# MisterVVP/poor-man-s-cache

Hardware: AMD Instinct MI355X
Metric: device-resident value compress+decompress GiB/s at 1/2/4/8 MI355X (higher is better)
Workload: dtype u8; 1 GPU; 10000000 x 1024 B values per GPU (JSON-slice), batched gzip level-9 compress + decompress, device-resident; outputs not checked in this run (--full checks every member); partition=MurmurHash3_x64_128('key'+i)[0] % 128 % n_gpus (NUM_SHARDS=128), parallelism=shard-partitioned x1, no collective

## Files before the change

poor-man-s-cache_amd/csrc/pmc_capi.hip:

```cpp
#include <hip/hip_runtime.h>

#include <vector>

#include <algorithm>
#include <atomic>
#include <cstdlib>
#include <cstdio>
#include <cstring>
#include <chrono>
#include <condition_variable>
#include <functional>
#include <mutex>
#include <string>
#include <thread>

#include <unistd.h>

#include "../../include/pmc_codec.h"
#include "pmc_device.hpp"
#include "pmc_kernels.hpp"

#define PMC_API extern "C" __attribute__((visibility("default")))

namespace pmc {
// ... 794 lines not shown
        e.cap_len = R.maxlen;
        e.wave_bytes = deflate_lv_emit_wave_bytes(R.maxlen);
        const uint64_t ew = std::max<uint64_t>(4, std::min<uint64_t>(
            {(uint64_t)(R.nv + 3) / 4 * 4, (uint64_t)ctx->cus * 4, std::max<uint64_t>(4, (8ull << 30) / e.wave_bytes / 4 * 4)}));
        r = ctx->lvemit.ensure(ew * e.wave_bytes);
        if (r) return r;
        e.scratch = (uint8_t *)ctx->lvemit.p;
        klaunch(ctx, PMC_K_DEFLATE_LARGE_EMIT, st, [&] {
            hipLaunchKernelGGL(deflate_lv_emit_kernel, dim3((unsigned)(ew / 4)), dim3(256), deflate_lv_emit_lds(4), st, e,
                               L);
        });
        hipError_t err = hipGetLastError();
        if (err != hipSuccess) {
            set_err(fast ? "fast large-value kernels" : "large-value kernels", err);
            return PMC_E_NO_DEVICE;
        }
        v0 = R.v1;
    }
    return PMC_OK;
}

static uint64_t split_chunk_budget() {
    static const uint64_t budget = (getenv("PMC_SPLIT_CHUNK_MB") ? (uint64_t)atoll(getenv("PMC_SPLIT_CHUNK_MB"))
                                                                 : 98304ull) << 20;
    return budget;
}

static int run_split_pass(pmc_ctx *ctx, DeflateArgs &a, const SplitPass &ps, uint32_t dD, hipStream_t st) {
    const uint64_t n = a.n, pcap = ps.pcap;
    const bool fastp = ps.fastp, dictp = ps.dictp;
    static const bool no_order = getenv("PMC_TREES_ORDER") && !atoi(getenv("PMC_TREES_ORDER"));
    const size_t tl_small = (size_t)(kTreesCap + 1) * 64 * 4, tl_1k = (size_t)(kTreesCap1K + 1) * 64 * 4;
    const size_t tl_big = (size_t)(kLCodes + 1) * 64 * 4;
    const uint32_t fcap = dictp ? 0u : front_cap_class(pcap);
    const uint64_t dcap = std::min<uint64_t>(((uint64_t)dD + ps.hi + 63) & ~(uint64_t)63, kDictSpan);
    const uint64_t fwb = dictp   ? deflate_front_fast_wave_bytes(dcap)
                         : fastp ? deflate_front_fast_wave_bytes(fcap ? fcap : pcap)
                                 : deflate_front_wave_bytes(fcap ? fcap : pcap);
    const uint64_t bwb = deflate_back_wave_bytes(pcap);
    a.dict = dictp ? (const uint8_t *)ctx->dict.p : nullptr;
    a.dict_len = dictp ? dD : 0u;
    a.front_cap = dictp ? (uint32_t)dcap : 0u;
    a.mtime = dictp ? ctx->dict_id : 0u;
    a.xfl = fastp ? 4u : 2u;
    const DeflateKernel fk = front_kernel(dictp, fastp, fcap);
    const Launch Lf = plan_lds(ctx, (const void *)fk, fwb, n, 0);
    const Launch Lb = plan_lds(ctx, (const void *)deflate_back_kernel, bwb, n, kBackTabBytes);
    const uint64_t chunk = split_chunk_of(n, split_chunk_budget(), pcap);
    const SplitLayout SL(pcap, chunk);
    uint8_t *p = (uint8_t *)ctx->split.p;
    a.cT = (uint32_t *)(p + SL.cT);
    a.cN = (uint32_t *)(p + SL.cN);
    a.cP = (uint32_t *)(p + SL.cP);
    a.cG = (uint32_t *)(p + SL.cG);
    a.cH = (uint16_t *)(p + SL.cH);
    a.cL = p + SL.cL;
    a.cB = (uint32_t *)(p + SL.cB);
    a.cC = (uint32_t *)(p + SL.cC);
    a.cD = (uint32_t *)(p + SL.cD);
    a.cZ = (uint32_t *)(p + SL.cZ);
    uint32_t *ord = (uint32_t *)(p + SL.ord), *obins = (uint32_t *)(p + SL.obins);
    a.cQ = (uint32_t *)(p + SL.cQ);
    a.min_len = ps.lo;
    a.lds_max_len = ps.hi;
    a.cap_len = pcap;
    a.front_batch = pcap <= 512 ? 4u : pcap <= 2048 ? 2u : 1u;
    for (uint64_t first = 0; first < n; first += chunk) {
        a.first = first;
        a.count = std::min<uint64_t>(chunk, n - first);
        const unsigned tb = (unsigned)((a.count + 63) / 64);
        a.wave_bytes = fwb;
        if (hipMemsetAsync(a.cQ, 0, 8, st) != hipSuccess) return PMC_E_NO_DEVICE;
        klaunch(ctx, PMC_K_DEFLATE_FRONT, st, [&] {
            const dim3 fg((unsigned)std::min<uint64_t>(Lf.blocks, (a.count + Lf.wpb - 1) / Lf.wpb));
            hipLaunchKernelGGL(fk, fg, dim3(64 * Lf.wpb), Lf.lds, st, a);
        });
        if (hipMemsetAsync(a.cD + a.count, 0, 4, st) != hipSuccess) return PMC_E_NO_DEVICE;
        a.cO = nullptr;
        if (!no_order && a.count >= 4096) {
            if (hipMemsetAsync(obins, 0, kOrderBins * 4, st) != hipSuccess) return PMC_E_NO_DEVICE;
            const unsigned ob = (unsigned)std::min<uint64_t>((a.count + 1023) / 1024, (uint64_t)ctx->cus * 4);
            klaunch(ctx, PMC_K_ORDER, st, [&] {
                hipLaunchKernelGGL(order_hist_kernel, dim3(ob), dim3(256), 0, st, (const uint32_t *)a.cZ, a.count, obins);
                hipLaunchKernelGGL(order_scan_kernel, dim3(1), dim3(1024), 0, st, obins);
                hipLaunchKernelGGL(order_scatter_kernel, dim3(ob), dim3(256), 0, st, (const uint32_t *)a.cZ, a.count,
                                   obins, ord);
            });
            a.cO = ord;
        }
        klaunch(ctx, PMC_K_DEFLATE_TREES, st, [&] {
            if (pcap <= 1024) hipLaunchKernelGGL(deflate_trees_kernel<kTreesCap1K>, dim3(tb), dim3(64), tl_1k, st, a);
            else hipLaunchKernelGGL(deflate_trees_kernel<kTreesCap>, dim3(tb), dim3(64), tl_small, st, a);
            hipLaunchKernelGGL(deflate_trees_kernel<kLCodes>, dim3(std::min<unsigned>(tb, 2u * (unsigned)ctx->cus)),
                               dim3(64), tl_big, st, a);
        });
        a.wave_bytes = bwb;
        a.back_nostage = pcap <= kNostageMaxLen ? 1u : 0u;
        if (a.back_nostage) klaunch(ctx, PMC_K_DEFLATE_BACK, st, [&] {
            const unsigned cb = (unsigned)std::min<uint64_t>((a.count + 511) / 512, (uint64_t)ctx->cus * 4);
            hipLaunchKernelGGL(crc32_batch_kernel, dim3(cb), dim3(512), 0, st, (const uint8_t *)a.src,
                               (const uint64_t *)(a.src_off + a.first), (const uint32_t *)(a.src_len + a.first),
                               a.count, a.cC);
        });
        klaunch(ctx, PMC_K_DEFLATE_BACK, st, [&] {
            hipLaunchKernelGGL(deflate_back_kernel,
                               dim3((unsigned)std::min<uint64_t>(Lb.blocks, (a.count + Lb.wpb - 1) / Lb.wpb)),
                               dim3(64 * Lb.wpb), Lb.lds, st, a);
// ... 1294 lines not shown
```

poor-man-s-cache_amd/csrc/pmc_deflate_split.hip:

```cpp
#include <hip/hip_runtime.h>

#include "pmc_device.hpp"
#include "pmc_kernels.hpp"

namespace pmc {


template <uint32_t CAPC>
__global__ void __launch_bounds__(256, 7) deflate_front_kernel(DeflateArgs a) {
    extern __shared__ __attribute__((aligned(16))) uint8_t lds[];
    const int wpb = blockDim.x / 64, wib = threadIdx.x / 64, l = lane_id();
    const uint64_t lcap = CAPC ? (uint64_t)CAPC : a.cap_len;
    uint8_t *base = lds + (uint64_t)wib * (CAPC ? front_layout(lcap).total : a.wave_bytes);
    const SmallLayout L = small_layout(lcap);
    const FrontLayout F = front_layout(lcap);
    SmallWave w;
    small_wave_init(w, base, L, a, nullptr);
    w.S = to_lds<uint16_t>(base + F.S);
    w.R = to_lds<uint16_t>(base + F.R);
    w.CN = to_lds<uint8_t>(base + F.cn);
    w.HC = to_lds<uint64_t>(base + F.hc);
    w.EV = to_lds<uint32_t>(base + F.ev);
    w.cnp = F.pkb;
    w.s12 = front_s12(lcap) ? 1u : 0u;
    w.lfreq = to_lds<uint32_t>(base + F.freq);
    w.dfreq = w.lfreq + 288;
    w.blfreq = w.dfreq + 32;
    const uint32_t kBatch = a.front_batch;
    uint32_t nx = l == 0 ? atomicAdd(a.cQ, kBatch) : 0u;
    for (;;) {
        const uint64_t g = readlane(nx, 0);
        if (g >= a.count) break;
        nx = l == 0 ? atomicAdd(a.cQ, kBatch) : 0u;
        const uint64_t vl = g + (uint64_t)l;
        const bool in = (uint32_t)l < kBatch && vl < a.count;
        const uint32_t myl = in ? a.src_len[a.first + vl] : 0u;
        const uint64_t myo = in ? a.src_off[a.first + vl] : 0u;
        uint64_t todo = ballot(myl != 0 && myl > a.min_len && myl <= a.lds_max_len);
        while (todo) {
            const int jj = __builtin_ctzll(todo);
            todo &= todo - 1;
            const uint64_t v = g + (uint64_t)jj, gv = a.first + v;
            const uint32_t len = readlane(myl, jj);
            w.tok = (PMC_GLB uint32_t *)(a.cT + v * a.cap_len);
#ifdef PMC_FAULT_LANE_ORDER
            w.fault_rev = (uint32_t)(gv & 1);
#endif
            const uint8_t *vsrc = a.src + readlane64(myo, jj);
            const uint32_t ntok = w.run_front(vsrc, len);
            if (ntok == kNtokRetry) {
                if (l == 0) {
                    a.cN[v] = kNtokRetry;
                    a.cZ[v] = 0;
                    atomicAdd(a.guard, 1u);
                }
                continue;
            }
            uint32_t nz = 0;
            for (int s = l; s < kLCodes + kDCodes; s += 64) {
                const uint32_t f = s < kLCodes ? w.lfreq[s] : w.dfreq[s - kLCodes];
                a.cH[v * kSplitRows + s] = (uint16_t)f;
                nz += (uint32_t)__builtin_popcountll(ballot(s < kLCodes && f != 0));
            }
            if (l == 0) {
                a.cN[v] = ntok < kSymsPerBlock ? ntok : kNtokMultiBlock;
                a.cZ[v] = nz;
            }
        }
    }
    small_wave_stamps_out(w, a);
}
template __global__ void deflate_front_kernel<0>(DeflateArgs);
template __global__ void deflate_front_kernel<1024>(DeflateArgs);
template __global__ void deflate_front_kernel<4096>(DeflateArgs);

template <int CAP>
struct LaneTrees {
    PMC_LDS uint32_t *hp;
    RegU16<kMaxBits + 1> blc;
    RegU16<kBLCodes> blf;
    const uint16_t *hist;
    uint8_t *lens;
    uint32_t *mg;
    bool deferred = false;

    __device__ uint32_t H(uint32_t i) const { return hp[i * 64]; }
    __device__ void setH(uint32_t i, uint32_t v) { hp[i * 64] = v; }

    __device__ void down(uint32_t k, uint32_t n) {
        const uint32_t v = H(k), kv = v >> 10;
        uint32_t j = k << 1;
        while (j <= n) {
            uint32_t x = H(j);
            if (j < n) {
                const uint32_t y = H(j + 1);
                if ((y >> 10) <= (x >> 10)) {
                    j++;
                    x = y;
                }
            }
            if (kv <= (x >> 10)) break;
            setH(k, x);
            k = j;
            j <<= 1;
        }
        setH(k, v);
    }

    __device__ static uint32_t xbits(int kind, uint32_t x) {
        return kind == 0 ? (x >= kLiterals + 1 ? len_extra_cf(x - (kLiterals + 1)) : 0u)
               : kind == 1 ? dist_extra_cf(x)
                           : (x == 16 ? 2u : x == 17 ? 3u : x == 18 ? 7u : 0u);
    }
    __device__ static uint32_t static_len(int kind, uint32_t x) {
        return kind == 1 ? 5u : x < 144 ? 8u : x < 256 ? 9u : x < 280 ? 7u : 8u;
    }
    template <class Freq>
    __device__ int build(Freq freq, int elems, uint32_t row0, int kind, int max_length, uint32_t &opt, uint32_t &stat,
                         PMC_GLB const uint16_t *grow = nullptr) {
        int heap_len = 0, max_code = -1;
        if (grow) {
            typedef uint32_t v4u __attribute__((ext_vector_type(4)));
            PMC_GLB const v4u *g4 = (PMC_GLB const v4u *)grow;
            const int nb = (elems + 31) / 32;
            v4u cur[4], nxt[4];
#pragma unroll
            for (int i = 0; i < 4; i++) cur[i] = i * 8 < elems ? g4[i] : v4u{0, 0, 0, 0};
            for (int b = 0; b < nb; b++) {
#pragma unroll
                for (int i = 0; i < 4; i++) {
                    const int q = (b + 1) * 4 + i;
                    nxt[i] = b + 1 < nb && q * 8 < elems ? g4[q] : v4u{0, 0, 0, 0};
                }
#pragma unroll
                for (int i = 0; i < 4; i++) {
#pragma unroll
                    for (int h = 0; h < 8; h++) {
                        const int nn = b * 32 + i * 8 + h;
                        const uint32_t f = nn < elems ? (cur[i][h >> 1] >> (16 * (h & 1))) & 0xffffu : 0u;
                        if (f) {
                            if (heap_len == CAP) {
                                deferred = true;
                                return -1;
                            }
                            setH(++heap_len, f << 15 | (uint32_t)nn);
                            max_code = nn;
                        }
                    }
                }
#pragma unroll
                for (int i = 0; i < 4; i++) cur[i] = nxt[i];
            }
        }
        for (int n0 = 0; !grow && n0 < elems; n0 += 8) {
            uint32_t f8[8];
#pragma unroll
            for (int k = 0; k < 8; k++) f8[k] = n0 + k < elems ? freq(n0 + k) : 0u;
#pragma unroll
            for (int k = 0; k < 8; k++) {
                if (f8[k]) {
                    if (heap_len == CAP) {
                        deferred = true;
                        return -1;
                    }
                    setH(++heap_len, f8[k] << 15 | (uint32_t)(n0 + k));
                    max_code = n0 + k;
                }
            }
        }
        while (heap_len < 2) {
            const int node = max_code < 2 ? ++max_code : 0;
            setH(++heap_len, 1u << 15 | (uint32_t)node);
            opt--;
            if (kind != 2) stat -= static_len(kind, (uint32_t)node);
        }
        for (int n = heap_len / 2; n >= 1; n--) down((uint32_t)n, (uint32_t)heap_len);
        uint32_t node = (uint32_t)elems, nm = 0;
        do {
            const uint32_t n = H(1);
            setH(1, H((uint32_t)heap_len));
            heap_len--;
            down(1, (uint32_t)heap_len);
            const uint32_t m = H(1);
            mg[(2 * nm) * 64] = n;
            mg[(2 * nm + 1) * 64] = m;
            nm++;
            const uint32_t kn = n >> 10, km = m >> 10, dn = kn & 31, dm = km & 31;
            const uint32_t d = (dn >= dm ? dn : dm) + 1;
            setH(1, ((((kn >> 5) + (km >> 5)) << 5) | d) << 10 | node);
            node++;
            down(1, (uint32_t)heap_len);
        } while (heap_len >= 2);
        const uint32_t K = nm;
        uint32_t overflow = 0;
        blc.zero();
        setH(K, 0);
        constexpr int kB = 8;
        uint32_t cur[2 * kB], nxt[2 * kB], nx2[2 * kB];
        auto fetch = [&](int hi, uint32_t *d) {
#pragma unroll
            for (int t = 0; t < kB; t++) {
                const int j = hi - 1 - t;
                d[2 * t] = j >= 0 ? mg[(2 * j + 1) * 64] : 0u;
                d[2 * t + 1] = j >= 0 ? mg[(2 * j) * 64] : 0u;
            }
        };
        fetch((int)K, cur);
        fetch((int)K - kB, nxt);
        for (int i0 = (int)K; i0 >= 1; i0 -= kB) {
            fetch(i0 - 2 * kB, nx2);
#pragma unroll
            for (int t = 0; t < kB; t++) {
                const int i = i0 - t;
                if (i < 1) break;
                const uint32_t L = H((uint32_t)i);
#pragma unroll
                for (int c = 0; c < 2; c++) {
                    const uint32_t key = cur[2 * t + c], x = key & 1023;
                    uint32_t bits = L + 1;
                    if (bits > (uint32_t)max_length) {
                        bits = (uint32_t)max_length;
                        overflow++;
                    }
                    if (x >= (uint32_t)elems) {
                        setH(x - (uint32_t)elems + 1, bits);
                    } else {
                        lens[row0 + x] = (uint8_t)bits;
                        blc.add(bits, 1);
                        const uint32_t f = key >> 15;
                        const uint32_t xb = xbits(kind, x);
                        opt += __umul24(f, bits + xb);
                        if (kind != 2) stat += __umul24(f, static_len(kind, x) + xb);
                    }
                }
            }
#pragma unroll
            for (int t = 0; t < 2 * kB; t++) {
                cur[t] = nxt[t];
                nxt[t] = nx2[t];
            }
        }
        if (overflow) {
            int ov = (int)overflow;
            do {
                int bits = max_length - 1;
                while (blc.get((uint32_t)bits) == 0) bits--;
                blc.add((uint32_t)bits, -1);
                blc.add((uint32_t)bits + 1, 2);
                blc.add((uint32_t)max_length, -1);
                ov -= 2;
            } while (ov > 0);
            uint32_t idx = 0;
            for (int bits = max_length; bits != 0; bits--) {
                uint32_t n = blc.get((uint32_t)bits);
                while (n != 0) {
                    const uint32_t key = mg[idx * 64], x = key & 1023;
                    idx++;
                    if (x >= (uint32_t)elems) continue;
                    const uint32_t cur = lens[row0 + x];
                    if (cur != (uint32_t)bits) {
                        opt += (uint32_t)((int32_t)bits - (int32_t)cur) * (key >> 15);
                        lens[row0 + x] = (uint8_t)bits;
                    }
                    n--;
                }
            }
        }
        return max_code;
    }

    __device__ void emit_header(int l_max, int d_max, int mbi, const uint32_t *blw, PMC_GLB uint32_t *row) {
        auto blen = [&](int s) -> uint32_t { return (blw[(12 + s) >> 2] >> (8 * ((12 + s) & 3))) & 0xffu; };
        uint64_t cnt = 0;
#pragma unroll
        for (int s = 0; s < kBLCodes; s++) {
            const uint32_t L = blen(s);
            cnt += L ? 1ull << (8 * L) : 0ull;
        }
        uint64_t nc = 0;
        uint32_t code = 0;
#pragma unroll
        for (int b = 1; b <= kMaxBLBits; b++) {
            code = (code + (uint32_t)((cnt >> (8 * (b - 1))) & 0xffu)) << 1;
            nc |= (uint64_t)code << (8 * b);
        }
        RegU16<kBLCodes> bc;
#pragma unroll
        for (int s = 0; s < kBLCodes; s++) {
            const uint32_t L = blen(s), c = (uint32_t)(nc >> (8 * L)) & 0xffu;
            nc += L ? 1ull << (8 * L) : 0ull;
            bc.set((uint32_t)s, L ? (__builtin_bitreverse32(c) >> (32 - L)) | L << 8 : 0u);
        }
        uint64_t acc = 0;
        uint32_t an = 0, wi = 1, total = 0;
        auto put = [&](uint32_t v, uint32_t n) {
            acc |= (uint64_t)v << an;
            an += n;
            total += n;
            if (an >= 32) {
                row[wi++] = (uint32_t)acc;
                acc >>= 32;
                an -= 32;
            }
        };
        auto send_code = [&](uint32_t sym) {
            const uint32_t e = bc.get(sym);
            put(e & 0xffu, e >> 8);
        };
        put((uint32_t)(l_max + 1 - 257), 5);
        put((uint32_t)d_max, 5);
        put((uint32_t)(mbi + 1 - 4), 4);
        for (int k = 0; k <= mbi; k++) put(bc.get(bl_order_cf(k)) >> 8, 3);
        for (int tr = 0; tr < 2; tr++) {
            const uint32_t row0 = tr ? (uint32_t)kLCodes : 0u;
            const int max_code = tr ? d_max : l_max;
            int prevlen = -1, nextlen = (int)lrow(row0), count = 0, max_count = 7, min_count = 4;
            if (nextlen == 0) max_count = 138, min_count = 3;
            int w0 = -8;
            uint64_t pk = 0;
            for (int n = 0; n <= max_code; n++) {
                const int curlen = nextlen, nx = n + 1;
// ... 46 lines not shown
#pragma unroll
        for (int i = 0; i < 20; i++) r[i] = *(PMC_GLB const v4u *)(lens + 16 * i);
#pragma unroll
        for (int i = 0; i < 20; i++) {
            hp[(4 * i + 0) * 64] = r[i].x;
            hp[(4 * i + 1) * 64] = r[i].y;
            hp[(4 * i + 2) * 64] = r[i].z;
            hp[(4 * i + 3) * 64] = r[i].w;
        }
    }

    __device__ void scan(uint32_t row0, int max_code) {
        int prevlen = -1, nextlen = (int)lrow(row0), count = 0, max_count = 7, min_count = 4;
        if (nextlen == 0) max_count = 138, min_count = 3;
        int w0 = -8;
        uint64_t pk = 0;
        for (int n = 0; n <= max_code; n++) {
            const int curlen = nextlen, nx = n + 1;
            if (nx <= max_code) {
                if (nx >= w0 + 8) {
                    w0 = nx & ~7;
                    pk = 0;
#pragma unroll
                    for (int k = 0; k < 8; k++)
                        pk |= (uint64_t)(w0 + k <= max_code ? lrow(row0 + (uint32_t)(w0 + k)) : 0u) << (8 * k);
                }
                nextlen = (int)((pk >> (8 * (nx - w0))) & 0xff);
            } else {
                nextlen = 0xffff;
            }
            if (++count < max_count && curlen == nextlen) {
                continue;
            }
            if (count < min_count) {
                blf.add((uint32_t)curlen, count);
            } else if (curlen != 0) {
                if (curlen != prevlen) blf.add((uint32_t)curlen, 1);
                blf.add(kRep3_6, 1);
            } else if (count <= 10) {
                blf.add(kRepz3_10, 1);
            } else {
                blf.add(kRepz11_138, 1);
            }
            count = 0;
            prevlen = curlen;
            if (nextlen == 0) max_count = 138, min_count = 3;
            else if (curlen == nextlen) max_count = 6, min_count = 3;
            else max_count = 7, min_count = 4;
        }
    }
};

template <int CAP>
__device__ void trees_value(const DeflateArgs &a, uint64_t v, uint64_t slot, PMC_LDS uint32_t *col) {
    const uint32_t len = a.src_len[a.first + v];
    if (len == 0 || len <= a.min_len || len > a.lds_max_len || a.cN[v] >= kNtokRetry) return;
    LaneTrees<CAP> t;
    t.hp = col;
    t.hist = a.cH + v * kSplitRows;
    t.lens = a.cL + v * kSplitRows;
    t.mg = a.cG + ((slot >> 6) * kMergeRows) * 64 + (slot & 63);
    for (uint32_t s = 0; s < kSplitRows; s += 16) *reinterpret_cast<uint4 *>(t.lens + s) = make_uint4(0, 0, 0, 0);
    uint32_t opt = 0, stat = 0;
    auto hist = [&](int s) -> uint32_t { return t.hist[s]; };
    const int l_max = t.build(hist, kLCodes, 0, 0, kMaxBits, opt, stat, (PMC_GLB const uint16_t *)t.hist);
    if (t.deferred) {
        a.cP[v] = kPlanDeferred;
        a.cD[atomicAdd(a.cD + a.count, 1u)] = (uint32_t)v;
        return;
    }
    {
        typedef uint32_t v4u __attribute__((ext_vector_type(4)));
        PMC_GLB const v4u *g4 = (PMC_GLB const v4u *)t.hist;
        static_assert(kLCodes * 2 == 35 * 16 + 12 && kDCodes == 30, "distance row at v4u 35, byte 12");
        static_assert(CAP >= 79, "heap slots 60..74 hold the staged distance frequencies, 0..79 the lengths row");
        v4u d5[5];
#pragma unroll
        for (int i = 0; i < 5; i++) d5[i] = g4[35 + i];
#pragma unroll
        for (int j = 3; j < 18; j++) t.hp[(57 + j) * 64] = d5[j >> 2][j & 3];
    }
    auto dhist = [&](int s) -> uint32_t { return (t.hp[(60 + (s >> 1)) * 64] >> (16 * (s & 1))) & 0xffffu; };
    const int d_max = t.build(dhist, kDCodes, kLCodes, 1, kMaxBits, opt, stat);
    t.blf.zero();
    t.stage_row();
    t.scan(0, l_max);
    t.scan(kLCodes, d_max);
    auto bfreq = [&](int s) -> uint32_t { return t.blf.get((uint32_t)s); };
    t.build(bfreq, kBLCodes, kLCodes + kDCodes, 2, kMaxBLBits, opt, stat);
    static_assert(kLCodes + kDCodes == 316 && kSplitRows >= 336, "bl lengths at row bytes 316..334");
    typedef uint32_t v4u __attribute__((ext_vector_type(4)));
    const v4u q0 = *(PMC_GLB const v4u *)(t.lens + 304), q1 = *(PMC_GLB const v4u *)(t.lens + 320);
    const uint32_t blw[8] = {q0.x, q0.y, q0.z, q0.w, q1.x, q1.y, q1.z, q1.w};
    int mbi = 2;
#pragma unroll
    for (int k = kBLCodes - 1; k >= 3; k--) {
        const int j = 12 + (int)bl_order_cf(k);
        if (mbi == 2 && ((blw[j >> 2] >> (8 * (j & 3))) & 0xffu) != 0) mbi = k;
    }
    opt += 3 * ((uint32_t)mbi + 1) + 5 + 5 + 4;
    uint32_t opt_lenb = (opt + 3 + 7) >> 3;
    const uint32_t static_lenb = (stat + 3 + 7) >> 3;
    if (static_lenb <= opt_lenb) opt_lenb = static_lenb;
    const uint32_t type = len + 4 <= opt_lenb ? 0u : static_lenb == opt_lenb ? 1u : 2u;
    const bool hdr = type == 2 && len > kHdrMinLen;
    a.cP[v] = type | (uint32_t)l_max << 2 | (uint32_t)d_max << 11 | (uint32_t)mbi << 16 | (hdr ? kPlanHdr : 0u);
    if (hdr) {
        t.stage_row();
        t.emit_header(l_max, d_max, mbi, blw, (PMC_GLB uint32_t *)(a.cB + v * kHdrWords));
    }
}

template <int CAP>
__global__ void __launch_bounds__(64) deflate_trees_kernel(DeflateArgs a) {
    extern __shared__ __attribute__((aligned(16))) uint32_t tl[];
    const uint32_t l = threadIdx.x;
    PMC_LDS uint32_t *col = to_lds<uint32_t>(tl + l);
    if (CAP != kLCodes) {
        const uint64_t vi = (uint64_t)blockIdx.x * 64 + l;
        if (vi < a.count) trees_value<CAP>(a, a.cO ? (uint64_t)a.cO[a.count - 1 - vi] : vi, vi, col);
    } else {
        const uint32_t nd = a.cD[a.count];
        for (uint32_t k = blockIdx.x * 64 + l; k < nd; k += gridDim.x * 64)
            trees_value<CAP>(a, a.cD[k], a.cD[k], col);
    }
}
template __global__ void deflate_trees_kernel<kTreesCap>(DeflateArgs);
template __global__ void deflate_trees_kernel<kTreesCap1K>(DeflateArgs);
template __global__ void deflate_trees_kernel<kLCodes>(DeflateArgs);

__global__ void __launch_bounds__(256, 5) deflate_back_kernel(DeflateArgs a) {
    extern __shared__ __attribute__((aligned(16))) uint8_t lds[];
    uint32_t *crc_tab = reinterpret_cast<uint32_t *>(lds);
    for (int k = threadIdx.x; k < 8 * 256; k += blockDim.x) crc_tab[k] = c_crc_slice8[k];
    __syncthreads();
    const int wpb = blockDim.x / 64, wib = threadIdx.x / 64, l = lane_id();
    uint8_t *base = lds + kBackTabBytes + (uint64_t)wib * a.wave_bytes;
    const SmallLayout L = small_layout(a.cap_len);
    const BackLayout B = back_layout(a.cap_len);
    SmallWave w;
    small_wave_init(w, base, L, a, crc_tab);
    w.outw = to_lds<uint32_t>(base + B.out);
    w.outb = to_lds<uint8_t>(base + B.out);
    w.out_words = (uint32_t)B.out_words;
    w.lcode = to_lds<uint32_t>(base + B.lcode);
    w.dcode = to_lds<uint32_t>(base + B.dcode);
    w.blcode = to_lds<uint32_t>(base + B.blcode);
    w.runs = to_lds<uint16_t>(base + B.runs);
    w.blfreq = to_lds<uint32_t>(base + B.blfreq);
    w.perm = to_lds<uint16_t>(base + B.perm);
    w.xfl = a.xfl;
    w.mtime = a.mtime;
    PMC_LDS uint8_t *Ls = to_lds<uint8_t>(base + B.ls);
    constexpr uint32_t kBatch = 16;
    uint32_t nx = l == 0 ? atomicAdd(a.cQ + 1, kBatch) : 0u;
    for (;;) {
        const uint64_t g = readlane(nx, 0);
        if (g >= a.count) break;
        nx = l == 0 ? atomicAdd(a.cQ + 1, kBatch) : 0u;
        const uint64_t vl = g + (uint64_t)l;
        const bool in = (uint32_t)l < kBatch && vl < a.count;
        const uint32_t myl = in ? a.src_len[a.first + vl] : 0u;
        const uint32_t myn = in ? a.cN[vl] : 0u, myp = in ? a.cP[vl] : 0u;
        const uint32_t myk = a.back_nostage && in ? a.cC[vl] : 0u;
        const uint64_t myo = in ? a.src_off[a.first + vl] : 0u, mydo = in ? a.dst_off[a.first + vl] : 0u;
        const uint32_t myc = in ? a.dst_cap[a.first + vl] : 0u;
        uint64_t todo = ballot(in && (a.min_len == 0 || myl > a.min_len) && myl <= a.lds_max_len);
        while (todo) {
            const int j = __builtin_ctzll(todo);
            todo &= todo - 1;
            const uint64_t v = g + (uint64_t)j, gv = a.first + v;
            const uint32_t len = readlane(myl, j);
            uint32_t pf = 0;
            if (todo) {
                const int j2 = __builtin_ctzll(todo);
                const uint64_t v2 = g + (uint64_t)j2;
                const uint32_t len2 = readlane(myl, j2), n2 = readlane(myn, j2);
// ... 52 lines not shown
```

poor-man-s-cache_amd/csrc/pmc_device.hpp:

```cpp
#pragma once
#include <hip/hip_runtime.h>
#include <stdint.h>

#include "pmc_trees.hpp"

namespace pmc {

constexpr int kWave = 64;

#define PMC_LDS __attribute__((address_space(3)))
#define PMC_GLB __attribute__((address_space(1)))
template <class T>
__device__ __forceinline__ PMC_LDS T *to_lds(void *p) {
    return (PMC_LDS T *)(p);
}
__device__ __forceinline__ uint32_t lds_add(PMC_LDS uint32_t *p, uint32_t v) {
    return __atomic_fetch_add(p, v, __ATOMIC_RELAXED);
}
__device__ __forceinline__ uint32_t lds_or(PMC_LDS uint32_t *p, uint32_t v) {
    return __atomic_fetch_or(p, v, __ATOMIC_RELAXED);
}
constexpr uint32_t kCrcPoly = 0xEDB88320u;
constexpr int kCrcShiftEntries = 4096;

extern __constant__ Tables c_tables;
extern __constant__ uint32_t c_crc_table[256];
extern __constant__ uint32_t c_crc_shift16[kCrcShiftEntries];
extern __constant__ uint32_t c_crc_shift64k[kCrcShiftEntries];
constexpr uint32_t kCrcPiece = 64;
constexpr uint32_t kCrcQuarterMax = 16 * kCrcPiece;
extern __constant__ uint32_t c_crc_slice8[8 * 256];
extern __constant__ uint32_t c_crc_zpiece[4 * 4 * 256];
extern __constant__ uint32_t c_crc_ones[kCrcQuarterMax + 1];

__device__ __forceinline__ int lane_id() { return (int)(threadIdx.x & 63); }
__device__ __forceinline__ uint32_t rfl(uint32_t v) { return __builtin_amdgcn_readfirstlane(v); }
__device__ __forceinline__ int rfl(int v) { return __builtin_amdgcn_readfirstlane(v); }
__device__ __forceinline__ uint64_t rfl64(uint64_t v) {
    uint32_t lo = rfl((uint32_t)v), hi = rfl((uint32_t)(v >> 32));
    return ((uint64_t)hi << 32) | lo;
}

__device__ __forceinline__ void wave_sync() {
    __builtin_amdgcn_fence(__ATOMIC_RELEASE, "wavefront");
    __builtin_amdgcn_wave_barrier();
    __builtin_amdgcn_fence(__ATOMIC_ACQUIRE, "wavefront");
}
__device__ __forceinline__ void wave_sync_global() {
    __builtin_amdgcn_fence(__ATOMIC_RELEASE, "workgroup");
    __builtin_amdgcn_wave_barrier();
    __builtin_amdgcn_fence(__ATOMIC_ACQUIRE, "workgroup");
}

__device__ __forceinline__ uint64_t ballot(bool p) { return __ballot(p); }

__device__ __forceinline__ uint32_t wave_max_u32(uint32_t v) {
// ... 41 lines not shown
    v += (uint32_t)__builtin_amdgcn_update_dpp(0, (int)v, 0x142, 0xa, 0xf, false);
    v += (uint32_t)__builtin_amdgcn_update_dpp(0, (int)v, 0x143, 0xc, 0xf, false);
    return v;
}
__device__ __forceinline__ uint32_t wave_incl_max_dpp(uint32_t v) {
    uint32_t t;
    t = (uint32_t)__builtin_amdgcn_update_dpp(0, (int)v, 0x111, 0xf, 0xf, false);
    v = t > v ? t : v;
    t = (uint32_t)__builtin_amdgcn_update_dpp(0, (int)v, 0x112, 0xf, 0xf, false);
    v = t > v ? t : v;
    t = (uint32_t)__builtin_amdgcn_update_dpp(0, (int)v, 0x114, 0xf, 0xf, false);
    v = t > v ? t : v;
    t = (uint32_t)__builtin_amdgcn_update_dpp(0, (int)v, 0x118, 0xf, 0xf, false);
    v = t > v ? t : v;
    t = (uint32_t)__builtin_amdgcn_update_dpp(0, (int)v, 0x142, 0xa, 0xf, false);
    v = t > v ? t : v;
    t = (uint32_t)__builtin_amdgcn_update_dpp(0, (int)v, 0x143, 0xc, 0xf, false);
    v = t > v ? t : v;
    return v;
}
__device__ __forceinline__ uint32_t dpp_row_max(uint32_t v) {
    uint32_t t;
    t = (uint32_t)__builtin_amdgcn_mov_dpp((int)v, 0xB1, 0xF, 0xF, false);
    v = t > v ? t : v;
    t = (uint32_t)__builtin_amdgcn_mov_dpp((int)v, 0x4E, 0xF, 0xF, false);
    v = t > v ? t : v;
    t = (uint32_t)__builtin_amdgcn_mov_dpp((int)v, 0x141, 0xF, 0xF, false);
    v = t > v ? t : v;
    t = (uint32_t)__builtin_amdgcn_mov_dpp((int)v, 0x140, 0xF, 0xF, false);
    v = t > v ? t : v;
    return v;
}
__device__ __forceinline__ uint32_t wave_max_dpp(uint32_t v) {
    v = dpp_row_max(v);
    uint32_t a = (uint32_t)__builtin_amdgcn_readlane((int)v, 0), b = (uint32_t)__builtin_amdgcn_readlane((int)v, 16);
    uint32_t c = (uint32_t)__builtin_amdgcn_readlane((int)v, 32), d = (uint32_t)__builtin_amdgcn_readlane((int)v, 48);
    a = a > b ? a : b;
    c = c > d ? c : d;
    return a > c ? a : c;
}
__device__ __forceinline__ uint32_t readlane(uint32_t v, int l) {
    return (uint32_t)__builtin_amdgcn_readlane((int)v, l);
}
__device__ __forceinline__ uint64_t readlane64(uint64_t v, int l) {
    return (uint64_t)readlane((uint32_t)(v >> 32), l) << 32 | readlane((uint32_t)v, l);
}
__device__ __forceinline__ uint32_t writelane(uint32_t old, uint32_t v, int l) {
    return lane_id() == l ? v : old;
}
__device__ __forceinline__ uint32_t popc_lt(uint64_t mask) {
    return (uint32_t)__builtin_amdgcn_mbcnt_hi((uint32_t)(mask >> 32), __builtin_amdgcn_mbcnt_lo((uint32_t)mask, 0));
}

template <int N>
struct RegU16 {
    static constexpr int kW = (N + 1) / 2;
    uint32_t w[kW];
    __device__ __forceinline__ void zero() {
#pragma unroll
        for (int j = 0; j < kW; j++) w[j] = 0;
    }
    __device__ __forceinline__ uint32_t get(uint32_t i) const {
        uint32_t x = 0;
#pragma unroll
        for (int j = 0; j < kW; j++) x = (i >> 1) == (uint32_t)j ? w[j] : x;
        return (x >> ((i & 1u) * 16)) & 0xffffu;
    }
    __device__ __forceinline__ void add(uint32_t i, int32_t v) {
        const uint32_t d = (uint32_t)v << ((i & 1u) * 16);
#pragma unroll
        for (int j = 0; j < kW; j++) w[j] += (i >> 1) == (uint32_t)j ? d : 0u;
    }
    __device__ __forceinline__ void set(uint32_t i, uint32_t v) {
        const uint32_t sh = (i & 1u) * 16;
#pragma unroll
        for (int j = 0; j < kW; j++)
            w[j] = (i >> 1) == (uint32_t)j ? (w[j] & ~(0xffffu << sh)) | (v & 0xffffu) << sh : w[j];
    }
};

__device__ __forceinline__ uint32_t multmodp(uint32_t a, uint32_t b) {
    uint32_t p = 0;
#pragma unroll 8
    for (int k = 31; k >= 0; k--) {
        p ^= ((a >> k) & 1u) ? b : 0u;
        b = (b >> 1) ^ (kCrcPoly & (0u - (b & 1u)));
    }
    return p;
}

__device__ __forceinline__ uint32_t crc_shift_chunks(uint32_t d) {
    uint32_t k = c_crc_shift16[d & (kCrcShiftEntries - 1)];
    if (d >= (uint32_t)kCrcShiftEntries) k = multmodp(k, c_crc_shift64k[d >> 12]);
    return k;
}

template <class BytePtr, class TabPtr>
__device__ inline uint32_t wave_crc32(BytePtr buf, uint32_t len, TabPtr tab) {
    uint32_t nchunks = (len + 15) >> 4;
    uint32_t acc = 0;
    for (uint32_t d = (uint32_t)lane_id(); d < nchunks; d += 64) {
        int64_t end = (int64_t)len - 16 * (int64_t)d;
        int64_t beg = end - 16;
        uint32_t c = 0;
        if (beg <= 0) {
            beg = 0;
            c = 0xFFFFFFFFu;
        }
        for (int64_t k = beg; k < end; k++) c = tab[(c ^ buf[k]) & 0xff] ^ (c >> 8);
        acc ^= d ? multmodp(crc_shift_chunks(d), c) : c;
    }
    acc = wave_xor_u32(acc);
    if (len == 0) return 0;
    return ~acc;
}

struct CrcX8 {
    uint32_t v[16];
};
constexpr CrcX8 make_crc_x8() {
    CrcX8 t{};
    uint32_t p = 0x80000000u;
    for (int r = 0; r < 16; r++) {
        t.v[r] = p;
        for (int b = 0; b < 8; b++) p = (p >> 1) ^ ((p & 1u) ? kCrcPoly : 0u);
    }
    return t;
}
__device__ __forceinline__ uint32_t wave_xor_dpp(uint32_t v) {
    v ^= (uint32_t)__builtin_amdgcn_mov_dpp((int)v, 0xB1, 0xF, 0xF, false);
    v ^= (uint32_t)__builtin_amdgcn_mov_dpp((int)v, 0x4E, 0xF, 0xF, false);
    v ^= (uint32_t)__builtin_amdgcn_mov_dpp((int)v, 0x141, 0xF, 0xF, false);
// ... 40 lines not shown
```

poor-man-s-cache_amd/csrc/pmc_kernels.hpp:

```cpp
#pragma once
#include <hip/hip_runtime.h>
#include <stdint.h>

#include "pmc_plan.hpp"

namespace pmc {

constexpr int PMC_INVALID_INPUT_DEV = -999;
constexpr int PMC_Z_DATA_ERROR_DEV = -3;
constexpr int PMC_Z_BUF_ERROR_DEV = -5;
constexpr int PMC_E_CAPACITY_DEV = -101;
constexpr int PMC_E_ARG_DEV = -102;

constexpr uint32_t kSlabSyms = 16384;

struct DeflateArgs {
    const uint8_t *src;
    const uint64_t *src_off;
    const uint32_t *src_len;
    uint8_t *dst;
    const uint64_t *dst_off;
    const uint32_t *dst_cap;
    uint32_t *dst_len;
    int32_t *rc;
    uint64_t n;
    uint64_t cap_len;
    uint64_t lds_max_len;
    uint64_t wave_bytes;
    uint32_t *tokens;
    uint8_t *scratch;
    uint64_t *dbg;
    int32_t stop_after;
    uint64_t first, count;
    uint32_t *cT;
    uint32_t *cN;
    uint16_t *cH;
    uint8_t *cL;
    uint32_t *cB;
    uint32_t *cC;
    uint32_t back_nostage;
    uint32_t *cP;
    uint32_t *cG;
    uint32_t *cD;
    uint32_t *cZ;
    uint32_t *cO;
    uint32_t *cQ;
    uint64_t min_len;
    int32_t retry;
    uint32_t front_batch;
    uint32_t *guard;
    int32_t gate;
    uint32_t *rlist;
    uint32_t xfl = 2;
    uint32_t mtime = 0;
    const uint8_t *dict = nullptr;
    uint32_t dict_len = 0;
    uint32_t front_cap = 0;
};

__device__ inline void retry_push(const DeflateArgs &a, uint64_t v) {
    if (a.rlist) a.rlist[1 + atomicAdd(a.rlist, 1u)] = (uint32_t)v;
}

struct LargeArgs {
    const uint8_t *src;
    const uint64_t *src_off;
    const uint32_t *src_len;
    const uint32_t *lv_val;
    const uint64_t *lv_pbase;
    const uint32_t *lv_seg0;
    const uint32_t *lv_ch0;
    const uint32_t *seg_val;
    const uint64_t *seg_tok0;
    const uint32_t *ch_val;
    uint32_t nv, nseg, nch;
    uint32_t idx_crc;
    uint32_t *tmp, *S, *R;
    uint8_t *HC;
    uint32_t *hist;
    uint32_t *tok;
    uint32_t *map;
    uint32_t *seg_tok;
    int32_t *fail;
    uint32_t xfl;
    uint32_t idx_chunk;
};
__global__ void lv_select_kernel(const uint32_t *src_len, uint64_t n, uint64_t lo, uint64_t hi, uint32_t *out);
__global__ void lv_sort_hist_kernel(LargeArgs a, int pass);
__global__ void lv_sort_scan_kernel(LargeArgs a);
__global__ void lv_sort_scatter_kernel(LargeArgs a, int pass);
__global__ void lv_rank_kernel(LargeArgs a);
__global__ void lv_parse_kernel(LargeArgs a);
__global__ void lv_stitch_kernel(LargeArgs a);
__global__ void lv_fast_parse_kernel(DeflateArgs a, LargeArgs L);
uint64_t lv_fast_wave_bytes();
// ... 186 lines not shown
```

Before: 34.36 GiB/s.

## Store Huffman merge pairs in the LDS heap column instead of a global merge buffer

Moves the per-lane Huffman tree builder into a reusable LaneHeap struct. Merge pairs are now packed into freed heap slots in LDS rather than written to a separate global merge buffer (cG), which removes that scratch allocation and its global traffic. Code lengths are propagated by OR-ing depth bits into the parent slots. Cost terms are computed algebraically: the optimal length is the sum of internal node weights, and extra-bit and static costs are accumulated while leaves are pushed, replacing per-leaf multiply-adds in the length pass. The trade-off is extra LDS read-modify-write operations and more arithmetic at push time.

Result: no change. 34.61 GiB/s (median of 6 runs) (+0.7%).

```diff
diff --git a/poor-man-s-cache_amd/csrc/pmc_capi.hip b/poor-man-s-cache_amd/csrc/pmc_capi.hip
--- a/poor-man-s-cache_amd/csrc/pmc_capi.hip
+++ b/poor-man-s-cache_amd/csrc/pmc_capi.hip
@@ -870,7 +870,6 @@
     a.cT = (uint32_t *)(p + SL.cT);
     a.cN = (uint32_t *)(p + SL.cN);
     a.cP = (uint32_t *)(p + SL.cP);
-    a.cG = (uint32_t *)(p + SL.cG);
     a.cH = (uint16_t *)(p + SL.cH);
     a.cL = p + SL.cL;
     a.cB = (uint32_t *)(p + SL.cB);
diff --git a/poor-man-s-cache_amd/csrc/pmc_deflate_split.hip b/poor-man-s-cache_amd/csrc/pmc_deflate_split.hip
--- a/poor-man-s-cache_amd/csrc/pmc_deflate_split.hip
+++ b/poor-man-s-cache_amd/csrc/pmc_deflate_split.hip
@@ -74,199 +74,50 @@
 template __global__ void deflate_front_kernel<1024>(DeflateArgs);
 template __global__ void deflate_front_kernel<4096>(DeflateArgs);
 
+struct LdsCol {
+    PMC_LDS uint32_t *hp;
+    __device__ uint32_t get(uint32_t i) const { return hp[i * 64]; }
+    __device__ void set(uint32_t i, uint32_t v) { hp[i * 64] = v; }
+    __device__ void orr(uint32_t i, uint32_t v) { (void)lds_or(hp + i * 64, v); }
+};
+
 template <int CAP>
 struct LaneTrees {
     PMC_LDS uint32_t *hp;
-    RegU16<kMaxBits + 1> blc;
+    LaneHeap<CAP, LdsCol> heap;
     RegU16<kBLCodes> blf;
     const uint16_t *hist;
     uint8_t *lens;
-    uint32_t *mg;
-    bool deferred = false;
-
-    __device__ uint32_t H(uint32_t i) const { return hp[i * 64]; }
-    __device__ void setH(uint32_t i, uint32_t v) { hp[i * 64] = v; }
-
-    __device__ void down(uint32_t k, uint32_t n) {
-        const uint32_t v = H(k), kv = v >> 10;
-        uint32_t j = k << 1;
-        while (j <= n) {
-            uint32_t x = H(j);
-            if (j < n) {
-                const uint32_t y = H(j + 1);
-                if ((y >> 10) <= (x >> 10)) {
-                    j++;
-                    x = y;
-                }
-            }
-            if (kv <= (x >> 10)) break;
-            setH(k, x);
-            k = j;
-            j <<= 1;
-        }
-        setH(k, v);
-    }
-
-    __device__ static uint32_t xbits(int kind, uint32_t x) {
-        return kind == 0 ? (x >= kLiterals + 1 ? len_extra_cf(x - (kLiterals + 1)) : 0u)
-               : kind == 1 ? dist_extra_cf(x)
-                           : (x == 16 ? 2u : x == 17 ? 3u : x == 18 ? 7u : 0u);
-    }
-    __device__ static uint32_t static_len(int kind, uint32_t x) {
-        return kind == 1 ? 5u : x < 144 ? 8u : x < 256 ? 9u : x < 280 ? 7u : 8u;
-    }
+
     template <class Freq>
-    __device__ int build(Freq freq, int elems, uint32_t row0, int kind, int max_length, uint32_t &opt, uint32_t &stat,
-                         PMC_GLB const uint16_t *grow = nullptr) {
-        int heap_len = 0, max_code = -1;
-        if (grow) {
-            typedef uint32_t v4u __attribute__((ext_vector_type(4)));
-            PMC_GLB const v4u *g4 = (PMC_GLB const v4u *)grow;
-            const int nb = (elems + 31) / 32;
-            v4u cur[4], nxt[4];
-#pragma unroll
-            for (int i = 0; i < 4; i++) cur[i] = i * 8 < elems ? g4[i] : v4u{0, 0, 0, 0};
-            for (int b = 0; b < nb; b++) {
-#pragma unroll
-                for (int i = 0; i < 4; i++) {
-                    const int q = (b + 1) * 4 + i;
-                    nxt[i] = b + 1 < nb && q * 8 < elems ? g4[q] : v4u{0, 0, 0, 0};
-                }
-#pragma unroll
-                for (int i = 0; i < 4; i++) {
-#pragma unroll
-                    for (int h = 0; h < 8; h++) {
-                        const int nn = b * 32 + i * 8 + h;
-                        const uint32_t f = nn < elems ? (cur[i][h >> 1] >> (16 * (h & 1))) & 0xffffu : 0u;
-                        if (f) {
-                            if (heap_len == CAP) {
-                                deferred = true;
-                                return -1;
-                            }
-                            setH(++heap_len, f << 15 | (uint32_t)nn);
-                            max_code = nn;
-                        }
-                    }
-                }
-#pragma unroll
-                for (int i = 0; i < 4; i++) cur[i] = nxt[i];
-            }
-        }
-        for (int n0 = 0; !grow && n0 < elems; n0 += 8) {
-            uint32_t f8[8];
-#pragma unroll
-            for (int k = 0; k < 8; k++) f8[k] = n0 + k < elems ? freq(n0 + k) : 0u;
-#pragma unroll
-            for (int k = 0; k < 8; k++) {
-                if (f8[k]) {
-                    if (heap_len == CAP) {
-                        deferred = true;
-                        return -1;
-                    }
-                    setH(++heap_len, f8[k] << 15 | (uint32_t)(n0 + k));
-                    max_code = n0 + k;
-                }
-            }
-        }
-        while (heap_len < 2) {
-            const int node = max_code < 2 ? ++max_code : 0;
-            setH(++heap_len, 1u << 15 | (uint32_t)node);
-            opt--;
-            if (kind != 2) stat -= static_len(kind, (uint32_t)node);
-        }
-        for (int n = heap_len / 2; n >= 1; n--) down((uint32_t)n, (uint32_t)heap_len);
-        uint32_t node = (uint32_t)elems, nm = 0;
-        do {
-            const uint32_t n = H(1);
-            setH(1, H((uint32_t)heap_len));
-            heap_len--;
-            down(1, (uint32_t)heap_len);
-            const uint32_t m = H(1);
-            mg[(2 * nm) * 64] = n;
-            mg[(2 * nm + 1) * 64] = m;
-            nm++;
-            const uint32_t kn = n >> 10, km = m >> 10, dn = kn & 31, dm = km & 31;
-            const uint32_t d = (dn >= dm ? dn : dm) + 1;
-            setH(1, ((((kn >> 5) + (km >> 5)) << 5) | d) << 10 | node);
-            node++;
-            down(1, (uint32_t)heap_len);
-        } while (heap_len >= 2);
-        const uint32_t K = nm;
-        uint32_t overflow = 0;
-        blc.zero();
-        setH(K, 0);
-        constexpr int kB = 8;
-        uint32_t cur[2 * kB], nxt[2 * kB], nx2[2 * kB];
-        auto fetch = [&](int hi, uint32_t *d) {
-#pragma unroll
-            for (int t = 0; t < kB; t++) {
-                const int j = hi - 1 - t;
-                d[2 * t] = j >= 0 ? mg[(2 * j + 1) * 64] : 0u;
-                d[2 * t + 1] = j >= 0 ? mg[(2 * j) * 64] : 0u;
-            }
-        };
-        fetch((int)K, cur);
-        fetch((int)K - kB, nxt);
-        for (int i0 = (int)K; i0 >= 1; i0 -= kB) {
-            fetch(i0 - 2 * kB, nx2);
-#pragma unroll
-            for (int t = 0; t < kB; t++) {
-                const int i = i0 - t;
-                if (i < 1) break;
-                const uint32_t L = H((uint32_t)i);
-#pragma unroll
-                for (int c = 0; c < 2; c++) {
-                    const uint32_t key = cur[2 * t + c], x = key & 1023;
-                    uint32_t bits = L + 1;
-                    if (bits > (uint32_t)max_length) {
-                        bits = (uint32_t)max_length;
-                        overflow++;
-                    }
-                    if (x >= (uint32_t)elems) {
-                        setH(x - (uint32_t)elems + 1, bits);
-                    } else {
-                        lens[row0 + x] = (uint8_t)bits;
-                        blc.add(bits, 1);
-                        const uint32_t f = key >> 15;
-                        const uint32_t xb = xbits(kind, x);
-                        opt += __umul24(f, bits + xb);
-                        if (kind != 2) stat += __umul24(f, static_len(kind, x) + xb);
-                    }
-                }
-            }
-#pragma unroll
-            for (int t = 0; t < 2 * kB; t++) {
-                cur[t] = nxt[t];
-                nxt[t] = nx2[t];
-            }
-        }
-        if (overflow) {
-            int ov = (int)overflow;
-            do {
-                int bits = max_length - 1;
-                while (blc.get((uint32_t)bits) == 0) bits--;
-                blc.add((uint32_t)bits, -1);
-                blc.add((uint32_t)bits + 1, 2);
-                blc.add((uint32_t)max_length, -1);
-                ov -= 2;
-            } while (ov > 0);
-            uint32_t idx = 0;
-            for (int bits = max_length; bits != 0; bits--) {
-                uint32_t n = blc.get((uint32_t)bits);
-                while (n != 0) {
-                    const uint32_t key = mg[idx * 64], x = key & 1023;
-                    idx++;
-                    if (x >= (uint32_t)elems) continue;
-                    const uint32_t cur = lens[row0 + x];
-                    if (cur != (uint32_t)bits) {
-                        opt += (uint32_t)((int32_t)bits - (int32_t)cur) * (key >> 15);
-                        lens[row0 + x] = (uint8_t)bits;
-                    }
-                    n--;
-                }
-            }
-        }
-        return max_code;
+    __device__ int build_row(Freq freq, int elems, int kind, int max_length, uint32_t &opt, uint32_t &stat,
+                             PMC_GLB const uint16_t *grow) {
+        typedef uint32_t v4u __attribute__((ext_vector_type(4)));
+        PMC_GLB const v4u *g4 = (PMC_GLB const v4u *)grow;
+        const int nb = (elems + 31) / 32;
+        v4u cur[4], nxt[4];
+        heap.begin();
+#pragma unroll
+        for (int i = 0; i < 4; i++) cur[i] = i * 8 < elems ? g4[i] : v4u{0, 0, 0, 0};
+        for (int b = 0; b < nb; b++) {
+#pragma unroll
+            for (int i = 0; i < 4; i++) {
+                const int q = (b + 1) * 4 + i;
+                nxt[i] = b + 1 < nb && q * 8 < elems ? g4[q] : v4u{0, 0, 0, 0};
+            }
+#pragma unroll
+            for (int i = 0; i < 4; i++) {
+                const int n0 = b * 32 + i * 8;
+                uint32_t f8[8];
+#pragma unroll
+                for (int h = 0; h < 8; h++) f8[h] = n0 + h < elems ? (cur[i][h >> 1] >> (16 * (h & 1))) & 0xffffu : 0u;
+                heap.push8(kind, f8, (uint32_t)n0);
+            }
+            if (heap.deferred) return -1;
+#pragma unroll
+            for (int i = 0; i < 4; i++) cur[i] = nxt[i];
+        }
+        return heap.finish(freq, elems, lens, kind, max_length, opt, stat);
     }
 
     __device__ void emit_header(int l_max, int d_max, int mbi, const uint32_t *blw, PMC_GLB uint32_t *row) {
@@ -419,19 +270,18 @@
 };
 
 template <int CAP>
-__device__ void trees_value(const DeflateArgs &a, uint64_t v, uint64_t slot, PMC_LDS uint32_t *col) {
+__device__ void trees_value(const DeflateArgs &a, uint64_t v, PMC_LDS uint32_t *col) {
     const uint32_t len = a.src_len[a.first + v];
     if (len == 0 || len <= a.min_len || len > a.lds_max_len || a.cN[v] >= kNtokRetry) return;
     LaneTrees<CAP> t;
-    t.hp = col;
+    t.hp = t.heap.col.hp = col;
     t.hist = a.cH + v * kSplitRows;
     t.lens = a.cL + v * kSplitRows;
-    t.mg = a.cG + ((slot >> 6) * kMergeRows) * 64 + (slot & 63);
     for (uint32_t s = 0; s < kSplitRows; s += 16) *reinterpret_cast<uint4 *>(t.lens + s) = make_uint4(0, 0, 0, 0);
     uint32_t opt = 0, stat = 0;
     auto hist = [&](int s) -> uint32_t { return t.hist[s]; };
-    const int l_max = t.build(hist, kLCodes, 0, 0, kMaxBits, opt, stat, (PMC_GLB const uint16_t *)t.hist);
-    if (t.deferred) {
+    const int l_max = t.build_row(hist, kLCodes, 0, kMaxBits, opt, stat, (PMC_GLB const uint16_t *)t.hist);
+    if (t.heap.deferred) {
         a.cP[v] = kPlanDeferred;
         a.cD[atomicAdd(a.cD + a.count, 1u)] = (uint32_t)v;
         return;
@@ -448,13 +298,13 @@
         for (int j = 3; j < 18; j++) t.hp[(57 + j) * 64] = d5[j >> 2][j & 3];
     }
     auto dhist = [&](int s) -> uint32_t { return (t.hp[(60 + (s >> 1)) * 64] >> (16 * (s & 1))) & 0xffffu; };
-    const int d_max = t.build(dhist, kDCodes, kLCodes, 1, kMaxBits, opt, stat);
+    const int d_max = t.heap.build(dhist, kDCodes, t.lens + kLCodes, 1, kMaxBits, opt, stat);
     t.blf.zero();
     t.stage_row();
     t.scan(0, l_max);
     t.scan(kLCodes, d_max);
     auto bfreq = [&](int s) -> uint32_t { return t.blf.get((uint32_t)s); };
-    t.build(bfreq, kBLCodes, kLCodes + kDCodes, 2, kMaxBLBits, opt, stat);
+    t.heap.build(bfreq, kBLCodes, t.lens + (kLCodes + kDCodes), 2, kMaxBLBits, opt, stat);
     static_assert(kLCodes + kDCodes == 316 && kSplitRows >= 336, "bl lengths at row bytes 316..334");
     typedef uint32_t v4u __attribute__((ext_vector_type(4)));
     const v4u q0 = *(PMC_GLB const v4u *)(t.lens + 304), q1 = *(PMC_GLB const v4u *)(t.lens + 320);
@@ -485,11 +335,11 @@
     PMC_LDS uint32_t *col = to_lds<uint32_t>(tl + l);
     if (CAP != kLCodes) {
         const uint64_t vi = (uint64_t)blockIdx.x * 64 + l;
-        if (vi < a.count) trees_value<CAP>(a, a.cO ? (uint64_t)a.cO[a.count - 1 - vi] : vi, vi, col);
+        if (vi < a.count) trees_value<CAP>(a, a.cO ? (uint64_t)a.cO[a.count - 1 - vi] : vi, col);
     } else {
         const uint32_t nd = a.cD[a.count];
         for (uint32_t k = blockIdx.x * 64 + l; k < nd; k += gridDim.x * 64)
-            trees_value<CAP>(a, a.cD[k], a.cD[k], col);
+            trees_value<CAP>(a, a.cD[k], col);
     }
 }
 template __global__ void deflate_trees_kernel<kTreesCap>(DeflateArgs);
diff --git a/poor-man-s-cache_amd/csrc/pmc_device.hpp b/poor-man-s-cache_amd/csrc/pmc_device.hpp
--- a/poor-man-s-cache_amd/csrc/pmc_device.hpp
+++ b/poor-man-s-cache_amd/csrc/pmc_device.hpp
@@ -2,6 +2,7 @@
 #include <hip/hip_runtime.h>
 #include <stdint.h>
 
+#include "pmc_lane_trees.hpp"
 #include "pmc_trees.hpp"
 
 namespace pmc {
@@ -149,32 +150,6 @@
     return (uint32_t)__builtin_amdgcn_mbcnt_hi((uint32_t)(mask >> 32), __builtin_amdgcn_mbcnt_lo((uint32_t)mask, 0));
 }
 
-template <int N>
-struct RegU16 {
-    static constexpr int kW = (N + 1) / 2;
-    uint32_t w[kW];
-    __device__ __forceinline__ void zero() {
-#pragma unroll
-        for (int j = 0; j < kW; j++) w[j] = 0;
-    }
-    __device__ __forceinline__ uint32_t get(uint32_t i) const {
-        uint32_t x = 0;
-#pragma unroll
-        for (int j = 0; j < kW; j++) x = (i >> 1) == (uint32_t)j ? w[j] : x;
-        return (x >> ((i & 1u) * 16)) & 0xffffu;
-    }
-    __device__ __forceinline__ void add(uint32_t i, int32_t v) {
-        const uint32_t d = (uint32_t)v << ((i & 1u) * 16);
-#pragma unroll
-        for (int j = 0; j < kW; j++) w[j] += (i >> 1) == (uint32_t)j ? d : 0u;
-    }
-    __device__ __forceinline__ void set(uint32_t i, uint32_t v) {
-        const uint32_t sh = (i & 1u) * 16;
-#pragma unroll
-        for (int j = 0; j < kW; j++)
-            w[j] = (i >> 1) == (uint32_t)j ? (w[j] & ~(0xffffu << sh)) | (v & 0xffffu) << sh : w[j];
-    }
-};
 
 __device__ __forceinline__ uint32_t multmodp(uint32_t a, uint32_t b) {
     uint32_t p = 0;
diff --git a/poor-man-s-cache_amd/csrc/pmc_kernels.hpp b/poor-man-s-cache_amd/csrc/pmc_kernels.hpp
--- a/poor-man-s-cache_amd/csrc/pmc_kernels.hpp
+++ b/poor-man-s-cache_amd/csrc/pmc_kernels.hpp
@@ -40,7 +40,6 @@
     uint32_t *cC;
     uint32_t back_nostage;
     uint32_t *cP;
-    uint32_t *cG;
     uint32_t *cD;
     uint32_t *cZ;
     uint32_t *cO;
diff --git a/poor-man-s-cache_amd/csrc/pmc_lane_trees.hpp b/poor-man-s-cache_amd/csrc/pmc_lane_trees.hpp
--- /dev/null
+++ b/poor-man-s-cache_amd/csrc/pmc_lane_trees.hpp
@@ -0,0 +1,209 @@
+#pragma once
+#include <stdint.h>
+
+#include "pmc_trees.hpp"
+
+#ifndef PMC_HDI
+#if defined(__HIPCC__)
+#define PMC_HDI __host__ __device__ __forceinline__
+#else
+#define PMC_HDI inline
+#endif
+#endif
+
+namespace pmc {
+
+template <int N>
+struct RegU16 {
+    static constexpr int kW = (N + 1) / 2;
+    uint32_t w[kW];
+    PMC_HDI void zero() {
+#pragma unroll
+        for (int j = 0; j < kW; j++) w[j] = 0;
+    }
+    PMC_HDI uint32_t get(uint32_t i) const {
+        uint32_t x = 0;
+#pragma unroll
+        for (int j = 0; j < kW; j++) x = (i >> 1) == (uint32_t)j ? w[j] : x;
+        return (x >> ((i & 1u) * 16)) & 0xffffu;
+    }
+    PMC_HDI void add(uint32_t i, int32_t v) {
+        const uint32_t d = (uint32_t)v << ((i & 1u) * 16);
+#pragma unroll
+        for (int j = 0; j < kW; j++) w[j] += (i >> 1) == (uint32_t)j ? d : 0u;
+    }
+    PMC_HDI void set(uint32_t i, uint32_t v) {
+        const uint32_t sh = (i & 1u) * 16;
+#pragma unroll
+        for (int j = 0; j < kW; j++)
+            w[j] = (i >> 1) == (uint32_t)j ? (w[j] & ~(0xffffu << sh)) | (v & 0xffffu) << sh : w[j];
+    }
+};
+
+PMC_HDI uint32_t lane_mul24(uint32_t a, uint32_t b) {
+#if defined(__HIP_DEVICE_COMPILE__)
+    return __umul24(a, b);
+#else
+    return a * b;
+#endif
+}
+
+template <int CAP, class Col>
+struct LaneHeap {
+    static_assert(CAP >= 2 && CAP <= kLCodes, "a tree has 2 .. 286 leaves");
+    static_assert(2 * kLCodes - 1 < 1024 && kMaxBits < 16, "node ids take 10 bits, a length 4");
+    Col col;
+    RegU16<kMaxBits + 1> blc;
+    bool deferred = false;
+    int heap_len, max_code;
+    uint32_t xsum, ssum;
+
+    PMC_HD uint32_t H(uint32_t i) const { return col.get(i); }
+    PMC_HD void setH(uint32_t i, uint32_t v) { col.set(i, v); }
+
+    PMC_HD void down(uint32_t k, uint32_t n) {
+        const uint32_t v = H(k), kv = v >> 10;
+        uint32_t j = k << 1;
+        while (j <= n) {
+            uint32_t x = H(j);
+            if (j < n) {
+                const uint32_t y = H(j + 1);
+                if ((y >> 10) <= (x >> 10)) {
+                    j++;
+                    x = y;
+                }
+            }
+            if (kv <= (x >> 10)) break;
+            setH(k, x);
+            k = j;
+            j <<= 1;
+        }
+        setH(k, v);
+    }
+
+    PMC_HD static uint32_t xbits(int kind, uint32_t x) {
+        return kind == 0 ? (x >= kLiterals + 1 ? len_extra_cf(x - (kLiterals + 1)) : 0u)
+               : kind == 1 ? dist_extra_cf(x)
+                           : (x == 16 ? 2u : x == 17 ? 3u : x == 18 ? 7u : 0u);
+    }
+    PMC_HD static uint32_t static_len(int kind, uint32_t x) {
+        return kind == 1 ? 5u : x < 144 ? 8u : x < 256 ? 9u : x < 280 ? 7u : 8u;
+    }
+
+    PMC_HD void begin() {
+        heap_len = 0, max_code = -1;
+        xsum = ssum = 0;
+    }
+    PMC_HD void push_leaf(uint32_t f, uint32_t sym) {
+        if (heap_len < CAP) setH((uint32_t)++heap_len, f << 15 | sym);
+        else deferred = true;
+        max_code = (int)sym;
+    }
+    PMC_HD void push8(int kind, const uint32_t *f8, uint32_t n0) {
+        static_assert(144 % 8 == 0 && kLiterals % 8 == 0 && 280 % 8 == 0, "static lit/len lengths change at multiples of 8");
+        uint32_t g = 0;
+#pragma unroll
+        for (uint32_t k = 0; k < 8; k++) {
+            const uint32_t f = f8[k], sym = n0 + k;
+            if (f == 0) continue;
+            push_leaf(f, sym);
+            if (kind == 0) {
+                g += f;
+                if (sym >= kLiterals + 1 + 8) xsum += lane_mul24(f, len_extra_cf(sym - (kLiterals + 1)));
+            } else {
+                xsum += lane_mul24(f, xbits(kind, sym));
+                if (kind == 1) ssum += lane_mul24(f, static_len(kind, sym));
+            }
+        }
+        if (kind == 0) ssum += lane_mul24(g, static_len(kind, n0));
+    }
+
+    template <class Freq, class Lens>
+    PMC_HD int finish(Freq freq, int elems, Lens lens, int kind, int max_length, uint32_t &opt, uint32_t &stat) {
+        while (heap_len < 2) {
+            const int node = max_code < 2 ? ++max_code : 0;
+            setH((uint32_t)++heap_len, 1u << 15 | (uint32_t)node);
+            opt--;
+        }
+        const uint32_t k = (uint32_t)heap_len;
+        for (int n = heap_len / 2; n >= 1; n--) down((uint32_t)n, (uint32_t)heap_len);
+        uint32_t node = (uint32_t)elems, wsum = 0;
+        do {
+            const uint32_t n = H(1);
+            setH(1, H((uint32_t)heap_len));
+            heap_len--;
+            down(1, (uint32_t)heap_len);
+            const uint32_t m = H(1);
+            setH((uint32_t)heap_len + 1, (n & 1023) | (m & 1023) << 10);
+            const uint32_t kn = n >> 10, km = m >> 10, dn = kn & 31, dm = km & 31;
+            const uint32_t d = (dn >= dm ? dn : dm) + 1, fs = (kn >> 5) + (km >> 5);
+            wsum += fs;
+            setH(1, ((fs << 5) | d) << 10 | node);
+            node++;
+            down(1, (uint32_t)heap_len);
+        } while (heap_len >= 2);
+        uint32_t overflow = 0;
+        blc.zero();
+        for (uint32_t s = 2; s <= k; s++) {
+            const uint32_t w = H(s);
+            uint32_t bits = (w >> 20) + 1;
+            if (bits > (uint32_t)max_length) {
+                bits = (uint32_t)max_length;
+                overflow += 2;
+            }
+#pragma unroll
+            for (int c = 0; c < 2; c++) {
+                const uint32_t x = (c == 0 ? w >> 10 : w) & 1023;
+                if (x >= (uint32_t)elems) {
+                    col.orr(k - (x - (uint32_t)elems), bits << 20);
+                } else {
+                    lens[x] = (uint8_t)bits;
+                    blc.add(bits, 1);
+                }
+            }
+        }
+        if (overflow) {
+            int ov = (int)overflow;
+            do {
+                int bits = max_length - 1;
+                while (blc.get((uint32_t)bits) == 0) bits--;
+                blc.add((uint32_t)bits, -1);
+                blc.add((uint32_t)bits + 1, 2);
+                blc.add((uint32_t)max_length, -1);
+                ov -= 2;
+            } while (ov > 0);
+            uint32_t idx = 0, fl = 0;
+            for (int bits = max_length; bits != 0; bits--) {
+                uint32_t n = blc.get((uint32_t)bits);
+                while (n != 0 && idx < 2 * (k - 1)) {
+                    const uint32_t w = H(k - (idx >> 1)), x = (idx & 1 ? w >> 10 : w) & 1023;
+                    idx++;
+                    if (x >= (uint32_t)elems) continue;
+                    lens[x] = (uint8_t)bits;
+                    fl += lane_mul24(freq((int)x), (uint32_t)bits);
+                    n--;
+                }
+            }
+            opt += fl + xsum;
+        } else {
+            opt += wsum + xsum;
+        }
+        if (kind != 2) stat += ssum + xsum;
+        return max_code;
+    }
+
+    template <class Freq, class Lens>
+    PMC_HD int build(Freq freq, int elems, Lens lens, int kind, int max_length, uint32_t &opt, uint32_t &stat) {
+        begin();
+        for (int n0 = 0; n0 < elems; n0 += 8) {
+            uint32_t f8[8];
+#pragma unroll
+            for (int k = 0; k < 8; k++) f8[k] = n0 + k < elems ? freq(n0 + k) : 0u;
+            push8(kind, f8, (uint32_t)n0);
+            if (deferred) return -1;
+        }
+        return finish(freq, elems, lens, kind, max_length, opt, stat);
+    }
+};
+
+}
```
